# wadewilliamsw1234/Multi-level-Indoor-SLAM

Measured on AMD Instinct MI355X. Metric: keyframes gated/sec (VPR+kNN+LightGlue verify), higher is better.
Workload: dtype bf16

## Files before the change

### include/mlgate.h

```cpp
#ifndef MLGATE_H
#define MLGATE_H

#include <stddef.h>
#include <stdint.h>

#ifdef __cplusplus
extern "C" {
#endif

#define MLG_OK 0
#define MLG_EINVAL (-1)
#define MLG_EHIP (-2)
#define MLG_ENOMEM (-3)

#define MLG_VIT_DEPTH 12
#define MLG_VIT_EMBED 768
#define MLG_VIT_PATCH_K 768

#define MLG_ABI_VERSION 3
#define MLG_STRUCT_INIT(T) {(uint32_t)sizeof(T), (uint32_t)MLG_ABI_VERSION}
int mlg_abi_version(void);
const char* mlg_strerror(int status);

typedef struct mlg_vit_block {
// ... 263 lines not shown

typedef struct mlg_lg_block {
    const uint16_t* Wqkv; const float* bqkv;
    const uint16_t* Wout; const float* bout;
    const uint16_t* Wf1;  const float* bf1;
    const float* ln_g;    const float* ln_b;
    const uint16_t* Wf2;  const float* bf2;
} mlg_lg_block;
typedef struct mlg_lg_weights {
    uint32_t struct_size, abi_version;
    const float* Wr;
    mlg_lg_block self[9], cross[9];
    const uint16_t* Wfinal[9]; const float* bfinal[9];
    const float* wmatch[9];    const float* bmatch[9];
    const float* wconf[8];     const float* bconf[8];
    const float* ones;
} mlg_lg_weights;
size_t mlg_lightglue_workspace_bytes(int P, int kmax);
int mlg_lightglue(const mlg_lg_weights* w, const float* keypoints, const float* descriptors, const int32_t* counts,
                  int F, int kmax, const int32_t* pair_a, const int32_t* pair_b, int P, float depth_confidence,
                  float width_confidence, float filter_threshold, int pruning_min_kpts, void* workspace,
                  size_t workspace_bytes, int32_t* matches, float* scores, int32_t* num_matches, int32_t* stop_layer,
                  void* stream);

int mlg_lg_orient_matches(const int32_t* matches, const float* scores, const int32_t* num_matches,
                          const int32_t* rows, const uint8_t* swap, int P, int kmax, int32_t* matches_out,
                          float* scores_out, int32_t* num_out, void* stream);

int mlg_dbg_lg_trace_begin(void* dev_buf, size_t bytes);
int mlg_dbg_lg_trace_end(int32_t* tags, int32_t* counts, int max_entries);
int mlg_dbg_fill_lds(uint32_t pattern, void* sink, void* stream);
int mlg_dbg_fill_regs(uint32_t pattern, void* stream);
int mlg_dbg_ransac_poison_nsol(int on, int value);
int mlg_dbg_ffn_trace(void* host, size_t bytes);
int mlg_dbg_att_trace(void* host, size_t bytes);

typedef struct mlg_sg_weights {
    uint32_t struct_size, abi_version;
    const float* kenc_w[3]; const float* kenc_b[3];
    const uint16_t* kenc_w4; const float* kenc_b4;
    const uint16_t* kenc_w5; const float* kenc_b5;
    mlg_lg_block layer[18];
    const uint16_t* Wfinal; const float* bfinal;
    float bin_score;
} mlg_sg_weights;
size_t mlg_superglue_workspace_bytes(int P, int kmax);
int mlg_superglue(const mlg_sg_weights* w, const float* keypoints, const float* scores, const float* descriptors,
                  const int32_t* counts, int F, int kmax, int W, int H, const int32_t* pair_a, const int32_t* pair_b,
                  int P, int sinkhorn_iterations, float match_threshold, void* workspace, size_t workspace_bytes,
                  int32_t* matches, float* match_scores, int32_t* num_matches, void* stream);

size_t mlg_ransac_workspace_bytes(int P, long S_total, int hypotheses);
int mlg_ransac_epipolar(const float* kp1, const float* kp2, const int32_t* offsets, int P, long S_total,
                        const double* K, int k_stride, double threshold, int hypotheses, uint64_t seed,
                        void* workspace, size_t workspace_bytes, double* model, uint8_t* mask, int32_t* inliers,
                        double* pose, int32_t* status, void* stream);
int mlg_recover_pose(const float* kp1, const float* kp2, const int32_t* offsets, int P, const double* K,
                     int k_stride, const double* E, const uint8_t* mask, double* pose, void* stream);

#define MLG_LOFTR_NCONV 21
typedef struct {
    const uint16_t* w;
    const uint16_t* wmerge;
    const uint16_t* w1;
    const uint16_t* w2;
    const float *ln1_g, *ln1_b, *ln2_g, *ln2_b;
// ... 80 lines not shown
```

### multi-level-indoor-slam_amd/csrc/ransac.hip

```cpp
#include "common.h"
#include "kernels.h"
#include "ws_carve.h"

#define RS_FN __host__ __device__ static inline
#define RS_CONST static __constant__ const
#include "rs_math.h"

namespace {

#define RS_HD __host__ __device__

constexpr int MAXSOL = 10;
constexpr int RS_CHUNK = 1024;
constexpr int RS_ROUND1 = 256;

__device__ __forceinline__ int nsol_at(const int8_t* __restrict__ nsol, size_t i) {
    return min(max((int)nsol[i], 0), MAXSOL);
}


template <int MR>
RS_HD bool null_space9(double (&A)[MR][9], double (&N)[9 - MR][9]) {
    int piv_col[MR];
    int r = 0;
    for (int c = 0; c < 9 && r < MR; ++c) {
        int best = r;
        double bv = fabs(A[r][c]);
        for (int i = r + 1; i < MR; ++i)
            if (fabs(A[i][c]) > bv) { bv = fabs(A[i][c]); best = i; }
        if (bv < 1e-12) continue;
        if (best != r)
            for (int j = 0; j < 9; ++j) { double t = A[r][j]; A[r][j] = A[best][j]; A[best][j] = t; }
        const double inv = 1.0 / A[r][c];
        for (int j = 0; j < 9; ++j) A[r][j] *= inv;
        for (int i = 0; i < MR; ++i)
            if (i != r) {
                const double f = A[i][c];
                if (f != 0.0)
                    for (int j = 0; j < 9; ++j) A[i][j] -= f * A[r][j];
            }
        piv_col[r++] = c;
    }
    if (r < MR) return false;
    bool is_piv[9] = {false, false, false, false, false, false, false, false, false};
    for (int i = 0; i < MR; ++i) is_piv[piv_col[i]] = true;
    int k = 0;
    for (int f = 0; f < 9; ++f) {
// ... 480 lines not shown
        }
        if (__all(done)) break;
    }
    bool real = r < n && fabs(zi) <= 1e-7 * fmax(1.0, fabs(zr));
    double x = zr;
    if (real) {
#pragma unroll
        for (int pass = 0; pass < 2; ++pass) {
            double f = 0.0, df = 0.0;
#pragma unroll
            for (int i = 10; i >= 0; --i)
                if (i <= n) { df = df * x + f; f = f * x + c[i]; }
            if (df != 0.0) {
                const double xn = x - f / df;
                if (isfinite(xn)) x = xn;
            }
        }
    }
    int nn = 0;
#pragma unroll
    for (int j = 0; j < 10; ++j) {
        const double v = __shfl(x, gl + j, 64);
        const int isr = __shfl((int)real, gl + j, 64);
        if (isr) {
#pragma unroll
            for (int i = 0; i < 10; ++i)
                if (i == nn) roots[i] = v;
            ++nn;
        }
    }
    return nn;
}

__device__ __forceinline__ bool hyp5_active(const PairInfo& pi, int h, int H, const int32_t* __restrict__ nsub, int p) {
    return h < H && (pi.mode == 5 ? h == 0 : h < nsub[p]);
}

__device__ __forceinline__ bool hyp5_null(const PairInfo& pi, const double4* __restrict__ ptsn,
                                          const int32_t* __restrict__ subsets, int p, int H, int h,
                                          double (&Nb)[4][9]) {
    double q1[5][2], q2[5][2];
    for (int i = 0; i < 5; ++i) {
        const int id = pi.mode == 5 ? i : subsets[((size_t)p * H + h) * 7 + i];
        const double4 q = ptsn[pi.start + id];
        q1[i][0] = q.x; q1[i][1] = q.y; q2[i][0] = q.z; q2[i][1] = q.w;
    }
    double A[5][9];
    for (int i = 0; i < 5; ++i) {
        const double x1 = q1[i][0], y1 = q1[i][1], x2 = q2[i][0], y2 = q2[i][1];
        A[i][0] = x2 * x1; A[i][1] = x2 * y1; A[i][2] = x2;
        A[i][3] = y2 * x1; A[i][4] = y2 * y1; A[i][5] = y2;
        A[i][6] = x1;      A[i][7] = y1;      A[i][8] = 1.0;
    }
    return null_space5_reg(A, Nb);
}

__global__ __launch_bounds__(64) void k_ransac_null5(const PairInfo* __restrict__ info, const double4* __restrict__ ptsn,
                                                     int H, const int32_t* __restrict__ subsets,
                                                     const int32_t* __restrict__ nsub, double* __restrict__ models,
                                                     int h0, int hn, const uint8_t* __restrict__ done) {
    const int p = blockIdx.y;
    const int h = h0 + blockIdx.x * 64 + threadIdx.x;
    if (h >= h0 + hn || (done && done[p])) return;
    const PairInfo pi = info[p];
    if (!(pi.mode == 1 || pi.mode == 5) || !hyp5_active(pi, h, H, nsub, p)) return;
    double Nb[4][9];
    const bool ok = hyp5_null(pi, ptsn, subsets, p, H, h, Nb);
    double* o = models + ((size_t)p * H + h) * MAXSOL * 9;
#pragma unroll
    for (int a = 0; a < 4; ++a)
#pragma unroll
        for (int k = 0; k < 9; ++k) o[9 * a + k] = Nb[a][k];
    o[36] = ok ? 1.0 : 0.0;
}

constexpr int HYP5_GS = 10, HYP5_GPW = 64 / HYP5_GS, HYP5_GPB = 4 * HYP5_GPW;
constexpr int SLOT_FLAG = 36, SLOT_POLY = 37, SLOT_MAT = 48;
constexpr double FLAG_POLY = 2.0;

template <class BX, class BY, class B1, class NB>
__device__ __forceinline__ int hyp5_models(const double (&zr)[10], int nz, BX bx, BY by, B1 b1, NB nb,
                                           double* __restrict__ out) {
    int ns = 0;
#pragma unroll
    for (int t = 0; t < 10; ++t) {
        if (t >= nz) continue;
        const double z = zr[t];
        double M[3][3];
#pragma unroll
        for (int i = 0; i < 3; ++i) {
            double vx = 0.0, vy = 0.0, v1 = 0.0;
#pragma unroll
            for (int d = 3; d >= 0; --d) { vx = vx * z + bx(i, d); vy = vy * z + by(i, d); }
#pragma unroll
            for (int d = 4; d >= 0; --d) v1 = v1 * z + b1(i, d);
            M[i][0] = vx; M[i][1] = vy; M[i][2] = v1;
        }
        double best[3] = {0.0, 0.0, 0.0}, bn = -1.0;
#pragma unroll
        for (int a = 0; a < 3; ++a) {
            const int b = (a + 1) % 3;
            const double cx = M[a][1] * M[b][2] - M[a][2] * M[b][1];
            const double cy = M[a][2] * M[b][0] - M[a][0] * M[b][2];
            const double cz = M[a][0] * M[b][1] - M[a][1] * M[b][0];
            const double n2 = cx * cx + cy * cy + cz * cz;
            if (n2 > bn) { bn = n2; best[0] = cx; best[1] = cy; best[2] = cz; }
        }
        if (!(fabs(best[2]) > 1e-300 * sqrt(fmax(bn, 1e-300)))) continue;
        const double x = best[0] / best[2], y = best[1] / best[2];
        if (!(fabs(x) < 1e300) || !(fabs(y) < 1e300)) continue;
        double e[9], nrm = 0.0;
#pragma unroll
        for (int k = 0; k < 9; ++k) {
            e[k] = x * nb(0, k) + y * nb(1, k) + z * nb(2, k) + nb(3, k);
            nrm += e[k] * e[k];
        }
        nrm = 1.0 / sqrt(nrm);
        double* Eo = out + ns * 9;
#pragma unroll
        for (int k = 0; k < 9; ++k) Eo[k] = e[k] * nrm;
        ++ns;
    }
    return ns;
}

__global__ __launch_bounds__(256) void k_ransac_hyp5(const PairInfo* __restrict__ info,
                                                     const double4* __restrict__ ptsn, int H,
                                                     const int32_t* __restrict__ subsets,
                                                     const int32_t* __restrict__ nsub, double* __restrict__ models,
                                                     int8_t* __restrict__ nsol, int h0,
                                                     const uint8_t* __restrict__ done) {
    constexpr int GS = HYP5_GS, GPW = HYP5_GPW, GPB = HYP5_GPB;
    __shared__ double snb[GPB][4][9];
    const int lane = threadIdx.x & 63, gw = lane / GS;
    const bool valid = gw < GPW;
    const int g = (threadIdx.x >> 6) * GPW + (valid ? gw : 0), r = lane - gw * GS, gl = gw * GS;
    const int p = blockIdx.y;
    const int h = h0 + blockIdx.x * GPB + g;
    if (done && done[p]) return;
    const PairInfo pi = info[p];
    const bool ess = pi.mode == 1 || pi.mode == 5;
    const bool act = valid && ess && hyp5_active(pi, h, H, nsub, p);
    if (!ess) return;
    bool ok = act;
    if (act) {
        const double* nb = models + ((size_t)p * H + h) * MAXSOL * 9;
        for (int i = r; i < 36; i += GS) snb[g][i / 9][i % 9] = nb[i];
        ok = nb[36] != 0.0;
    }
    __syncthreads();
    if (!valid) return;
#if defined(RS_ABLATE) && RS_ABLATE == 3
    if (act && r == 0) nsol[(size_t)p * H + h] = 0;
    return;
#endif
    auto ent = [&](int k, double* l) {
        for (int a = 0; a < 4; ++a) l[a] = snb[g][a][k];
    };
    double row[20];
#pragma unroll
    for (int j = 0; j < 20; ++j) row[j] = 0.0;
    if (ok && r == 0) {
        const int cof[3][5] = {{0, 4, 8, 5, 7}, {1, 3, 8, 5, 6}, {2, 3, 7, 4, 6}};
        const double sg[3] = {1.0, -1.0, 1.0};
#pragma unroll
        for (int t = 0; t < 3; ++t) {
            double l0[4], l1[4], l2[4], l3[4], l4[4];
            ent(cof[t][0], l0); ent(cof[t][1], l1); ent(cof[t][2], l2); ent(cof[t][3], l3); ent(cof[t][4], l4);
            double q[10];
#pragma unroll
            for (int s = 0; s < 10; ++s) q[s] = 0.0;
            q_fma(q, l1, l2, sg[t]);
            q_fma(q, l3, l4, -sg[t]);
            c_fma(row, q, l0);
        }
// ... 43 lines not shown
            if (ob > best) { best = ob; bl = jl; }
        }
        if (!(best > 1e-300)) ok = false;
        piv[c] = bl;
        double prow[20];
#pragma unroll
        for (int jj = c; jj < 20; ++jj) prow[jj] = __shfl(row[jj], gl + bl, 64);
        const double inv = ok ? 1.0 / prow[c] : 0.0;
        if (r == bl) {
#pragma unroll
            for (int jj = c; jj < 20; ++jj) row[jj] = prow[jj] * inv;
            used = true;
        } else {
            const double f = row[c] * inv;
#pragma unroll
            for (int jj = c; jj < 20; ++jj) row[jj] -= f * prow[jj];
        }
    }
    double bx[3][4], by[3][4], b1[3][5];
#pragma unroll
    for (int i = 0; i < 3; ++i) {
        double a4[10], a5[10];
#pragma unroll
        for (int k = 0; k < 10; ++k) {
            a4[k] = __shfl(row[10 + k], gl + piv[4 + 2 * i], 64);
            a5[k] = __shfl(row[10 + k], gl + piv[5 + 2 * i], 64);
        }
        bx[i][0] = a4[2]; bx[i][1] = a4[1] - a5[2]; bx[i][2] = a4[0] - a5[1]; bx[i][3] = -a5[0];
        by[i][0] = a4[5]; by[i][1] = a4[4] - a5[5]; by[i][2] = a4[3] - a5[4]; by[i][3] = -a5[3];
        b1[i][0] = a4[9]; b1[i][1] = a4[8] - a5[9]; b1[i][2] = a4[7] - a5[8]; b1[i][3] = a4[6] - a5[7];
        b1[i][4] = -a5[6];
    }
    if (!ok) {
        if (h < H && r == 0) nsol[(size_t)p * H + h] = 0;
        return;
    }
#if defined(RS_ABLATE) && RS_ABLATE == 2
    if (r == 0) nsol[(size_t)p * H + h] = (int8_t)(bx[0][0] > 1e300);
    return;
#endif
    double poly[11];
#pragma unroll
    for (int i = 0; i < 11; ++i) poly[i] = 0.0;
    {
        double t[8];
#pragma unroll
        for (int i = 0; i < 8; ++i) t[i] = 0.0;
        pmul_acc<4, 5>(t, by[1], b1[2], 1.0);
        pmul_acc<5, 4>(t, b1[1], by[2], -1.0);
        pmul_acc<4, 8>(poly, bx[0], t, 1.0);
#pragma unroll
        for (int i = 0; i < 8; ++i) t[i] = 0.0;
        pmul_acc<4, 5>(t, bx[1], b1[2], 1.0);
        pmul_acc<5, 4>(t, b1[1], bx[2], -1.0);
        pmul_acc<4, 8>(poly, by[0], t, -1.0);
        double u[7];
#pragma unroll
        for (int i = 0; i < 7; ++i) u[i] = 0.0;
        pmul_acc<4, 4>(u, bx[1], by[2], 1.0);
        pmul_acc<4, 4>(u, by[1], bx[2], -1.0);
        pmul_acc<5, 7>(poly, b1[0], u, 1.0);
    }
#if defined(RS_ABLATE) && RS_ABLATE == 1
    if (r == 0) nsol[(size_t)p * H + h] = (int8_t)(poly[3] > 1e300);
    return;
#endif
    if (r == 0) {
        double* o = models + ((size_t)p * H + h) * MAXSOL * 9;
#pragma unroll
        for (int i = 0; i < 11; ++i) o[SLOT_POLY + i] = poly[i];
#pragma unroll
        for (int i = 0; i < 3; ++i) {
#pragma unroll
            for (int d = 0; d < 4; ++d) {
                o[SLOT_MAT + 13 * i + d] = bx[i][d];
                o[SLOT_MAT + 13 * i + 4 + d] = by[i][d];
            }
#pragma unroll
            for (int d = 0; d < 5; ++d) o[SLOT_MAT + 13 * i + 8 + d] = b1[i][d];
        }
        o[SLOT_FLAG] = FLAG_POLY;
    }
}

__global__ __launch_bounds__(256) void k_ransac_roots5(const PairInfo* __restrict__ info, int H,
                                                       const int32_t* __restrict__ nsub, double* __restrict__ models,
                                                       int8_t* __restrict__ nsol, int h0,
                                                       const uint8_t* __restrict__ done) {
    constexpr int GS = HYP5_GS, GPW = HYP5_GPW, GPB = HYP5_GPB;
    __shared__ double2 szs[GPB][17];
    __shared__ double scoef[GPB][39 + 36];
    const int lane = threadIdx.x & 63, gw = lane / GS;
    const bool valid = gw < GPW;
    const int g = (threadIdx.x >> 6) * GPW + (valid ? gw : 0), r = lane - gw * GS, gl = gw * GS;
    const int p = blockIdx.y;
    const int h = h0 + blockIdx.x * GPB + g;
    if (done && done[p]) return;
    const PairInfo pi = info[p];
    if (!(pi.mode == 1 || pi.mode == 5) || !valid || !hyp5_active(pi, h, H, nsub, p)) return;
    double* o = models + ((size_t)p * H + h) * MAXSOL * 9;
    if (o[SLOT_FLAG] != FLAG_POLY) return;
    double* sc = scoef[g];
    for (int i = r; i < 39; i += GS) sc[i] = o[SLOT_MAT + i];
    for (int i = r; i < 36; i += GS) sc[39 + i] = o[i];
    double poly[11], zr[10];
#pragma unroll
    for (int i = 0; i < 11; ++i) poly[i] = o[SLOT_POLY + i];
    const int nz = real_roots10(poly, zr, r, gl, szs[g]);
    if (r != 0) return;
    __builtin_amdgcn_wave_barrier();
    nsol[(size_t)p * H + h] = (int8_t)hyp5_models(
        zr, nz, [&](int i, int d) { return sc[13 * i + d]; }, [&](int i, int d) { return sc[13 * i + 4 + d]; },
        [&](int i, int d) { return sc[13 * i + 8 + d]; }, [&](int a, int k) { return sc[39 + 9 * a + k]; }, o);
}

__global__ __launch_bounds__(64) void k_ransac_subsets(const PairInfo* __restrict__ info, int P, int H,
                                                       const float* __restrict__ kp1, const float* __restrict__ kp2,
                                                       int32_t* __restrict__ subsets, int32_t* __restrict__ nsub) {
    const int p = blockIdx.x * blockDim.x + threadIdx.x;
    if (p >= P) return;
    const PairInfo pi = info[p];
    if (pi.mode != 1 && pi.mode != 2) {
        nsub[p] = 0;
        return;
    }
    const int m = pi.mode == 1 ? 5 : 7;
    CvRng rng{~0ull};
    int32_t* out = subsets + (size_t)p * H * 7;
    int it = 0;
    for (; it < H; ++it) {
        int idx[7];
        float a[7][2], b[7][2];
        int iters = 0, i = 0;
        for (; iters < RANSAC_MAX_ATTEMPTS; ++iters) {
            for (i = 0; i < m;) {
                int v;
                for (;;) {
                    v = idx[i] = rng.uniform(0, pi.count);
                    int j = 0;
                    for (; j < i; ++j)
                        if (v == idx[j]) break;
                    if (j == i) break;
                }
                a[i][0] = kp1[2 * (pi.start + v)]; a[i][1] = kp1[2 * (pi.start + v) + 1];
                b[i][0] = kp2[2 * (pi.start + v)]; b[i][1] = kp2[2 * (pi.start + v) + 1];
                ++i;
            }
            if (m == 7 && (collinear_last(a, 7) || collinear_last(b, 7))) continue;
            break;
        }
        if (!(i == m && iters < RANSAC_MAX_ATTEMPTS)) break;
        for (int j = 0; j < m; ++j) out[it * 7 + j] = idx[j];
    }
    nsub[p] = it;
}

__global__ __launch_bounds__(64) void k_ransac_hyp(const PairInfo* __restrict__ info, const double4* __restrict__ ptsn,
                                                   int H, uint64_t seed, const int32_t* __restrict__ subsets,
                                                   const int32_t* __restrict__ nsub, double* __restrict__ models,
                                                   int8_t* __restrict__ nsol, int h0, const uint8_t* __restrict__ done) {
    const int p = blockIdx.y;
    const int h = h0 + blockIdx.x * blockDim.x + threadIdx.x;
    if (h >= H || (done && done[p])) return;
    const PairInfo pi = info[p];
    double* out = models + ((size_t)p * H + h) * MAXSOL * 9;
    if (pi.mode == 1 || pi.mode == 5) return;
    const bool direct = pi.mode == 4;
    if (pi.mode == 0 || (direct && h > 0)) {
        nsol[(size_t)p * H + h] = 0;
        return;
    }
    int idx[7];
    if (direct) {
        for (int i = 0; i < 7; ++i) idx[i] = i;
    } else if (pi.mode == 2) {
        if (h >= nsub[p]) {
            nsol[(size_t)p * H + h] = 0;
            return;
        }
        for (int i = 0; i < 7; ++i) idx[i] = subsets[((size_t)p * H + h) * 7 + i];
    } else {
        uint64_t st = splitmix(seed ^ (uint64_t)h * 0x632BE59BD9B4E019ull);
        for (int i = 0; i < 7; ++i) {
            int v;
            bool dup;
            do {
                st = splitmix(st);
                v = (int)((st >> 11) % (uint64_t)pi.count);
                dup = false;
                for (int j = 0; j < i; ++j) dup |= idx[j] == v;
            } while (dup);
            idx[i] = v;
        }
    }
    double q1[7][2], q2[7][2];
    for (int i = 0; i < 7; ++i) {
        const double4 q = ptsn[pi.start + idx[i]];
        q1[i][0] = q.x; q1[i][1] = q.y; q2[i][0] = q.z; q2[i][1] = q.w;
    }
    double Fn[3 * 9];
    const int ns = solve_7pt(q1, q2, Fn);
    for (int s = 0; s < ns; ++s) denorm_F(Fn + s * 9, pi.T1, pi.T2, out + s * 9);
    nsol[(size_t)p * H + h] = (int8_t)ns;
}

__global__ __launch_bounds__(256) void k_ransac_score(const PairInfo* __restrict__ info, const double4* __restrict__ ptsn,
                                                      const double4* __restrict__ ptsr, int H,
                                                      const double* __restrict__ models,
                                                      const int8_t* __restrict__ nsol, float* __restrict__ score,
                                                      int h0, const uint8_t* __restrict__ done) {
    __shared__ double4 sp[RS_CHUNK];
    const int p = blockIdx.y;
    const int h = h0 + blockIdx.x * blockDim.x + threadIdx.x;
    if (done && done[p]) return;
    const PairInfo pi = info[p];
    if (pi.mode == 0) {
        if (h < H)
            for (int s = 0; s < MAXSOL; ++s) score[((size_t)p * H + h) * MAXSOL + s] = -INFINITY;
        return;
    }
    const bool ess = pi.mode == 1 || pi.mode == 5;
    const double4* src = (ess ? ptsn : ptsr) + pi.start;
    const int ns = h < H ? nsol_at(nsol, (size_t)p * H + h) : 0;
    int cnt[MAXSOL];
    for (int s = 0; s < MAXSOL; ++s) cnt[s] = 0;
    const float t2 = (float)pi.thr2;
    const double t2_hi = 0.5 * ((double)t2 + (double)nextafterf(t2, INFINITY));
    const double* mh = models + ((size_t)p * H + (h < H ? h : 0)) * MAXSOL * 9;
    if (pi.mode == 3) {
        for (int s = 0; s < MAXSOL; ++s) {
            float med = INFINITY;
            if (s < ns) {
                float e[16];
                for (int i = 0; i < pi.count; ++i) {
                    const double4 q = src[i];
                    e[i] = err_epiline(mh + s * 9, q.x, q.y, q.z, q.w);
                }
                for (int i = 1; i < pi.count; ++i) {
                    const float v = e[i];
                    int j = i - 1;
                    while (j >= 0 && e[j] > v) { e[j + 1] = e[j]; --j; }
                    e[j + 1] = v;
                }
                med = e[pi.count / 2];
            }
            if (h < H) score[((size_t)p * H + h) * MAXSOL + s] = s < ns ? -med : -INFINITY;
        }
        return;
    }
    for (int c0 = 0; c0 < pi.count; c0 += RS_CHUNK) {
        const int cn = min(RS_CHUNK, pi.count - c0);
        __syncthreads();
        for (int i = threadIdx.x; i < cn; i += blockDim.x) sp[i] = src[c0 + i];
        __syncthreads();
        for (int s = 0; s < ns; ++s) {
            double M[9];
            for (int k = 0; k < 9; ++k) M[k] = mh[s * 9 + k];
            int c = 0;
            if (ess) {
                for (int i = 0; i < cn; ++i) {
                    const double4 q = sp[i];
                    c += sampson_inlier(M, q.x, q.y, q.z, q.w, t2, t2_hi);
                }
            } else {
                for (int i = 0; i < cn; ++i) {
                    const double4 q = sp[i];
                    c += err_epiline(M, q.x, q.y, q.z, q.w) <= t2;
                }
            }
            cnt[s] += c;
        }
    }
    if (h < H)
        for (int s = 0; s < MAXSOL; ++s)
            score[((size_t)p * H + h) * MAXSOL + s] = s < ns ? (float)cnt[s] : -INFINITY;
}

RS_HD void jacobi3(double (&A)[3][3], double (&V)[3][3], double (&w)[3]) {
    for (int i = 0; i < 3; ++i)
        for (int j = 0; j < 3; ++j) V[i][j] = i == j ? 1.0 : 0.0;
    for (int sweep = 0; sweep < 50; ++sweep) {
        const double off = fabs(A[0][1]) + fabs(A[0][2]) + fabs(A[1][2]);
        if (off < 1e-300) break;
        for (int p = 0; p < 2; ++p)
            for (int q = p + 1; q < 3; ++q) {
                if (fabs(A[p][q]) < 1e-300) continue;
                const double th = (A[q][q] - A[p][p]) / (2.0 * A[p][q]);
                const double t = (th >= 0 ? 1.0 : -1.0) / (fabs(th) + sqrt(th * th + 1.0));
                const double c = 1.0 / sqrt(t * t + 1.0), s = t * c;
                for (int k = 0; k < 3; ++k) {
                    const double akp = A[k][p], akq = A[k][q];
                    A[k][p] = c * akp - s * akq;
                    A[k][q] = s * akp + c * akq;
                }
                for (int k = 0; k < 3; ++k) {
                    const double apk = A[p][k], aqk = A[q][k];
                    A[p][k] = c * apk - s * aqk;
                    A[q][k] = s * apk + c * aqk;
                }
                for (int k = 0; k < 3; ++k) {
                    const double vkp = V[k][p], vkq = V[k][q];
                    V[k][p] = c * vkp - s * vkq;
                    V[k][q] = s * vkp + c * vkq;
                }
            }
    }
    for (int i = 0; i < 3; ++i) w[i] = A[i][i];
}
// ... 81 lines not shown
    for (int i = 0; i < 4; ++i)
        for (int j = 0; j <= i; ++j) {
            double s = M[i][j];
            for (int k = 0; k < j; ++k) s -= L[i][k] * L[j][k];
            if (i == j) {
                L[i][i] = sqrt(fmax(s, 1e-300));
            } else {
                L[i][j] = s / L[j][j];
            }
        }
    double X[4] = {0.5, 0.5, 0.5, 0.5};
    for (int it = 0; it < 6; ++it) {
        double y[4];
        for (int i = 0; i < 4; ++i) {
            double s = X[i];
            for (int k = 0; k < i; ++k) s -= L[i][k] * y[k];
            y[i] = s / L[i][i];
        }
        for (int i = 3; i >= 0; --i) {
            double s = y[i];
            for (int k = i + 1; k < 4; ++k) s -= L[k][i] * X[k];
            X[i] = s / L[i][i];
        }
        double n = sqrt(X[0] * X[0] + X[1] * X[1] + X[2] * X[2] + X[3] * X[3]);
        for (int i = 0; i < 4; ++i) X[i] /= n;
    }
    if (!(X[2] * X[3] > 0)) return false;
    const double X0 = X[0] / X[3], X1 = X[1] / X[3], X2 = X[2] / X[3];
    if (!(X2 < dist)) return false;
    const double z2 = R[2][0] * X0 + R[2][1] * X1 + R[2][2] * X2 + t[2];
    return z2 > 0 && z2 < dist;
}

__global__ __launch_bounds__(256) void k_ransac_probe(const PairInfo* __restrict__ info, int P, int H, int H1,
                                                      const float* __restrict__ score,
                                                      const int8_t* __restrict__ nsol,
                                                      const int32_t* __restrict__ nsub, uint8_t* __restrict__ done) {
    const int p = blockIdx.x * blockDim.x + threadIdx.x;
    if (p >= P) return;
    const PairInfo pi = info[p];
    uint8_t d = 0;
    if (pi.mode == 1 || pi.mode == 2) {
        const int mp = pi.mode == 1 ? 5 : 7;
        const int ns_it = nsub[p], total = H * MAXSOL;
        int niters = H, max_good = 0;
        for (int it = 0; it < niters && it < ns_it && it < H1; ++it) {
            const int ns = nsol_at(nsol, (size_t)p * H + it);
            for (int s = 0; s < ns; ++s) {
                const int g = (int)score[(size_t)p * total + it * MAXSOL + s];
                if (g > max(max_good, mp - 1)) {
                    max_good = g;
                    niters = ransac_update_iters(RANSAC_CONFIDENCE, (double)(pi.count - g) / pi.count, mp, niters);
                }
            }
        }
        d = (niters <= H1 || ns_it <= H1) ? 1 : 0;
    }
    done[p] = d;
}

__global__ __launch_bounds__(256) void k_ransac_select(const PairInfo* __restrict__ info,
                                                       const double4* __restrict__ ptsn,
                                                       const double4* __restrict__ ptsr, int H,
                                                       const double* __restrict__ models,
                                                       const float* __restrict__ score, const int8_t* __restrict__ nsol,
                                                       const int32_t* __restrict__ nsub, double* __restrict__ model_out,
                                                       uint8_t* __restrict__ mask, int32_t* __restrict__ inliers,
                                                       int32_t* __restrict__ status) {
    const int p = blockIdx.x, tid = threadIdx.x;
    const PairInfo pi = info[p];
    __shared__ float bs[256];
    __shared__ int bi[256];
    __shared__ double Mb[9];
    __shared__ int cnt_sh;
    const int total = H * MAXSOL;
    if (pi.mode == 1 || pi.mode == 2) {
        if (tid == 0) {
            const int mp = pi.mode == 1 ? 5 : 7;
            const int ns_it = nsub[p];
            int niters = H, max_good = 0, bidx = -1;
            for (int it = 0; it < niters && it < ns_it; ++it) {
                const int ns = nsol_at(nsol, (size_t)p * H + it);
                for (int s = 0; s < ns; ++s) {
                    const int g = (int)score[(size_t)p * total + it * MAXSOL + s];
                    if (g > max(max_good, mp - 1)) {
                        max_good = g;
                        bidx = it * MAXSOL + s;
                        niters = ransac_update_iters(RANSAC_CONFIDENCE, (double)(pi.count - g) / pi.count, mp, niters);
                    }
// ... 101 lines not shown
    double nt[3] = {-tv[0], -tv[1], -tv[2]};
    int g[4] = {0, 0, 0, 0};
    for (int i = tid; i < S; i += 256) {
        if (!mask[s0 + i]) continue;
        const double x1 = (kp1[2 * (s0 + i)] - cx) / fx, y1 = (kp1[2 * (s0 + i) + 1] - cy) / fy;
        const double x2 = (kp2[2 * (s0 + i)] - cx) / fx, y2 = (kp2[2 * (s0 + i) + 1] - cy) / fy;
        g[0] += cheiral(R1, tv, x1, y1, x2, y2, 50.0);
        g[1] += cheiral(R2, tv, x1, y1, x2, y2, 50.0);
        g[2] += cheiral(R1, nt, x1, y1, x2, y2, 50.0);
        g[3] += cheiral(R2, nt, x1, y1, x2, y2, 50.0);
    }
    for (int k = 0; k < 4; ++k) atomicAdd(&good[k], g[k]);
    __syncthreads();
    if (tid == 0) {
        const int a = good[0], b = good[1], cc = good[2], d = good[3];
        int pick;
        if (a >= b && a >= cc && a >= d) pick = 0;
        else if (b >= a && b >= cc && b >= d) pick = 1;
        else if (cc >= a && cc >= b && cc >= d) pick = 2;
        else pick = 3;
        const double (*R)[3] = (pick & 1) ? R2 : R1;
        const double* tt = (pick & 2) ? nt : tv;
        double* T = pose + p * 16;
        for (int i = 0; i < 3; ++i) {
            for (int j = 0; j < 3; ++j) T[i * 4 + j] = R[i][j];
            T[i * 4 + 3] = tt[i];
        }
        T[12] = 0.0; T[13] = 0.0; T[14] = 0.0; T[15] = 1.0;
    }
}

bool g_poison_nsol = false;
int g_poison_value = 0;

__global__ __launch_bounds__(64) void k_ransac_poison_nsol(const PairInfo* __restrict__ info, int H,
                                                           const int32_t* __restrict__ nsub, int8_t* __restrict__ nsol,
                                                           int h0, int hn, const uint8_t* __restrict__ done, int value) {
    const int p = blockIdx.y;
    const int h = h0 + blockIdx.x * blockDim.x + threadIdx.x;
    if (h >= h0 + hn || h >= H || (done && done[p])) return;
    const int mode = info[p].mode;
    const bool unused = mode == 0 || ((mode == 4 || mode == 5) && h > 0) || ((mode == 1 || mode == 2) && h >= nsub[p]);
    if (unused) nsol[(size_t)p * H + h] = (int8_t)value;
}

struct RsBufs {
    PairInfo* info;
    double4 *ptsn, *ptsr;
    double* models;
    int8_t* nsol;
    float* score;
    int32_t *subsets, *nsub;
    uint8_t* done;
};

size_t rs_carve(int P, long S_total, int H, void* base, RsBufs* out) {
    WsCarver c(base);
    RsBufs b;
    const size_t PH = (size_t)P * H;
    b.info = c.take<PairInfo>((size_t)P);
    b.ptsn = c.take<double4>((size_t)S_total);
    b.ptsr = c.take<double4>((size_t)S_total);
    b.models = c.take<double>(9 * MAXSOL * PH);
    b.nsol = c.take<int8_t>(PH);
    b.score = c.take<float>(MAXSOL * PH);
    b.subsets = c.take<int32_t>(7 * PH);
    b.nsub = c.take<int32_t>((size_t)P);
    b.done = c.take<uint8_t>((size_t)P);
    if (out) *out = b;
    return c.total();
}

}

size_t mlg_ransac_ws_bytes(int P, long S_total, int H) {
    if (P <= 0 || S_total < 0 || H <= 0) return 0;
    return rs_carve(P, S_total, H, nullptr, nullptr);
}

int mlg_ransac_run(const float* kp1, const float* kp2, const int32_t* offs, int P, long S_total, const double* K,
                   int k_stride, double thr, int H, uint64_t seed, void* ws, size_t ws_bytes, double* model_out,
                   uint8_t* mask, int32_t* inliers, double* pose, int32_t* status, hipStream_t s) {
    if (P <= 0 || H <= 0 || H > (1 << 20) || !(thr > 0.0) || S_total < 0) return MLG_EINVAL;
    RsBufs b;
    if (rs_carve(P, S_total, H, ws, &b) > ws_bytes) return MLG_EINVAL;
    hipLaunchKernelGGL(k_ransac_prep, dim3(P), dim3(256), 0, s, kp1, kp2, offs, K, k_stride, thr, b.info, b.ptsn,
                       b.ptsr);
    MLG_LAUNCH_CHECK();
    hipLaunchKernelGGL(k_ransac_subsets, dim3((P + 63) / 64), dim3(64), 0, s, b.info, P, H, kp1, kp2, b.subsets,
                       b.nsub);
    MLG_LAUNCH_CHECK();
    const int H1 = std::min(H, RS_ROUND1);
    for (int round = 0; round < 2; ++round) {
        const int h0 = round ? H1 : 0, hn = round ? H - H1 : H1;
        const uint8_t* skip = round ? b.done : nullptr;
        if (hn <= 0) break;
        hipLaunchKernelGGL(k_ransac_hyp, dim3((hn + 63) / 64, P), dim3(64), 0, s, b.info, b.ptsn, H, seed, b.subsets,
                           b.nsub, b.models, b.nsol, h0, skip);
        MLG_LAUNCH_CHECK();
        hipLaunchKernelGGL(k_ransac_null5, dim3((hn + 63) / 64, P), dim3(64), 0, s, b.info, b.ptsn, H, b.subsets,
                           b.nsub, b.models, h0, hn, skip);
        MLG_LAUNCH_CHECK();
        hipLaunchKernelGGL(k_ransac_hyp5, dim3((hn + HYP5_GPB - 1) / HYP5_GPB, P), dim3(256), 0, s, b.info, b.ptsn, H,
                           b.subsets, b.nsub, b.models, b.nsol, h0, skip);
        MLG_LAUNCH_CHECK();
        hipLaunchKernelGGL(k_ransac_roots5, dim3((hn + HYP5_GPB - 1) / HYP5_GPB, P), dim3(256), 0, s, b.info, H, b.nsub,
                           b.models, b.nsol, h0, skip);
        MLG_LAUNCH_CHECK();
        if (g_poison_nsol) {
            hipLaunchKernelGGL(k_ransac_poison_nsol, dim3((hn + 63) / 64, P), dim3(64), 0, s, b.info, H, b.nsub, b.nsol,
                               h0, hn, skip, g_poison_value);
            MLG_LAUNCH_CHECK();
        }
        hipLaunchKernelGGL(k_ransac_score, dim3((hn + 255) / 256, P), dim3(256), 0, s, b.info, b.ptsn, b.ptsr, H,
                           b.models, b.nsol, b.score, h0, skip);
        MLG_LAUNCH_CHECK();
        if (round == 0 && H1 < H) {
            hipLaunchKernelGGL(k_ransac_probe, dim3((P + 255) / 256), dim3(256), 0, s, b.info, P, H, H1, b.score,
                               b.nsol, b.nsub, b.done);
            MLG_LAUNCH_CHECK();
        }
    }
    hipLaunchKernelGGL(k_ransac_select, dim3(P), dim3(256), 0, s, b.info, b.ptsn, b.ptsr, H, b.models, b.score, b.nsol,
                       b.nsub, model_out, mask, inliers, status);
    MLG_LAUNCH_CHECK();
    if (pose && K) {
        hipLaunchKernelGGL(k_recover_pose, dim3(P), dim3(256), 0, s, kp1, kp2, offs, K, k_stride, model_out, mask, pose,
                           status);
        MLG_LAUNCH_CHECK();
    }
    return MLG_OK;
}

int mlg_recover_pose_run(const float* kp1, const float* kp2, const int32_t* offs, int P, const double* K,
                         int k_stride, const double* E, const uint8_t* mask, double* pose, hipStream_t s) {
    if (P <= 0) return MLG_EINVAL;
    hipLaunchKernelGGL(k_recover_pose, dim3(P), dim3(256), 0, s, kp1, kp2, offs, K, k_stride, E, mask, pose,
                       (int32_t*)nullptr);
    MLG_LAUNCH_CHECK();
    return MLG_OK;
}

extern "C" int mlg_dbg_ransac_poison_nsol(int on, int value) {
    g_poison_nsol = on != 0;
    g_poison_value = value;
    return MLG_OK;
}
```

### multi-level-indoor-slam_amd/mlgate/_native.py

```python
import ctypes
import os

_HERE = os.path.dirname(os.path.abspath(__file__))
LIB_PATH = os.path.join(_HERE, "libmlgate.so")
TORCH_LIB_PATH = os.path.join(_HERE, "libmlgate_torch.so")
OPS = ("vit_forward_into", "dino_forward_into", "dino_weights_check", "salad_forward", "knn_gate", "knn_query", "row_normalize", "similarity", "xcorr_score", "xcorr_batch",
       "superpoint",
       "lightglue", "ransac_epipolar", "recover_pose", "resnet50", "loftr_features", "loftr_pack_tails", "loftr_coarse_layer", "loftr_match", "superglue", "pillow_resize_224", "plane_ransac", "proximity",
       "jpeg_pixels", "mixvpr_forward", "mixvpr_head", "mixvpr_preprocess", "vlad", "anyloc_forward", "kmeans_step",
       "crica_forward", "vit_trunk", "crica_pool", "crica_encoder",
       "weights_check", "prof_enable", "prof_reset", "prof_read")


c_int, c_long, c_size_t, c_float, c_double, c_void_p = (
    ctypes.c_int, ctypes.c_long, ctypes.c_size_t, ctypes.c_float, ctypes.c_double, ctypes.c_void_p)

EXPORTS = {
    "mlg_abi_version": (c_int, []),
    "mlg_strerror": (ctypes.c_char_p, [c_int]),
    "mlg_vit_workspace_bytes": (c_size_t, [c_int, c_int]),
    "mlg_vit_forward": (c_int, [c_void_p, c_void_p, c_int, c_int, c_int, c_int, c_long, c_int, c_int, c_void_p,
                                c_size_t, c_void_p, c_void_p, c_void_p]),
    "mlg_dino_workspace_bytes": (c_size_t, [c_int, c_int, c_int]),
    "mlg_dino_forward": (c_int, [c_void_p, c_void_p, c_int, c_int, c_int, c_int, c_long, c_int, c_int, c_void_p,
# ... 80 lines not shown
    "mlg_op_gemm_conv": (c_int, [c_void_p, c_int, c_void_p, c_void_p, c_void_p, c_int, c_void_p, c_int, c_void_p,
                                 c_int, c_int, c_int, c_int, c_int, c_int, c_float, c_void_p]),
    "mlg_op_gemm_conv_upadd": (c_int, [c_void_p, c_int, c_void_p, c_void_p, c_void_p, c_int, c_int, c_void_p, c_int,
                                       c_int, c_int, c_void_p]),
    "mlg_op_gemm_bias_relu": (c_int, [c_void_p, c_int, c_void_p, c_void_p, c_void_p, c_int, c_int, c_int, c_int,
                                      c_int, c_void_p]),
    "mlg_op_gemm_bias_add_relu": (c_int, [c_void_p, c_int, c_void_p, c_void_p, c_void_p, c_void_p, c_int, c_void_p,
                                          c_int, c_int, c_int, c_void_p]),
    "mlg_op_gemm_bias_f32_ld": (c_int, [c_void_p, c_int, c_void_p, c_void_p, c_void_p, c_int, c_int, c_int, c_int,
                                        c_void_p]),
    "mlg_op_gemm_bias_split": (c_int, [c_void_p, c_int, c_void_p, c_void_p, c_void_p, c_void_p, c_int, c_int, c_int,
                                       c_void_p]),
    "mlg_op_gemm_qkv": (c_int, [c_void_p] * 6 + [c_int, c_int, c_int, c_void_p]),
    "mlg_op_gemm_patch": (c_int, [c_void_p] * 5 + [c_int, c_int, c_int, c_void_p]),
    "mlg_op_gemm_sim_split_loftr": (c_int, [c_void_p, c_void_p, c_int, c_int, c_int, c_void_p, c_int, c_int, c_int,
                                            c_long, c_void_p]),
    "mlg_op_lg_ffn_ex": (c_int, [c_void_p, c_void_p, c_void_p, c_int, c_int] + [c_void_p] * 8 + [c_int]
                         + [c_void_p] * 5 + [c_float, c_float, c_void_p, c_void_p, c_void_p]),
    "mlg_op_preprocess_patches": (c_int, [c_void_p, c_int, c_int, c_int, c_int, c_long, c_int, c_void_p,
                                          c_void_p]),
    "mlg_prof_enable": (c_int, [c_int]),
    "mlg_prof_reset": (c_int, []),
    "mlg_prof_read": (c_int, [c_int, ctypes.POINTER(c_double), ctypes.POINTER(c_long)]),
    "mlg_prof_read_work": (c_int, [c_int, ctypes.POINTER(c_double)]),
    "mlg_lg_orient_matches": (c_int, [c_void_p] * 5 + [c_int, c_int] + [c_void_p] * 4),
    "mlg_xcorr_batch_workspace_bytes": (c_size_t, [c_int, c_int, c_int, c_int]),
    "mlg_xcorr_batch": (c_int, [c_void_p, c_int, c_int, c_int, c_void_p, c_void_p, c_int, c_void_p, c_size_t,
                                c_void_p, c_void_p]),
    "mlg_dbg_lg_trace_begin": (c_int, [c_void_p, c_size_t]),
    "mlg_dbg_lg_trace_end": (c_int, [c_void_p, c_void_p, c_int]),
    "mlg_dbg_fill_lds": (c_int, [ctypes.c_uint32, c_void_p, c_void_p]),
    "mlg_dbg_fill_regs": (c_int, [ctypes.c_uint32, c_void_p]),
    "mlg_dbg_ransac_poison_nsol": (c_int, [c_int, c_int]),
    "mlg_loftr_tails_bytes": (c_size_t, []),
    "mlg_loftr_pack_tails": (c_int, [c_void_p, c_void_p, c_void_p]),
    "mlg_op_loftr_coarse_layer_ws_bytes": (c_size_t, [c_int, c_int]),
    "mlg_op_loftr_coarse_layer": (c_int, [c_void_p, c_int, c_int, c_void_p, c_void_p, c_int, c_int, c_void_p, c_size_t,
                                          c_void_p]),
    "mlg_png_info": (c_int, [c_void_p, c_size_t, c_void_p, c_void_p, c_void_p, c_void_p]),
    "mlg_png_decode_bgr": (c_int, [c_void_p, c_void_p, c_int, c_void_p, c_int, c_int, c_int, c_void_p]),
    "mlg_png_load_bgr": (c_int, [c_void_p, c_int, c_void_p, c_int, c_int, c_int, c_void_p]),
    "mlg_jpeg_info": (c_int, [c_void_p, c_size_t, c_void_p]),
    "mlg_jpeg_coef_bytes": (c_size_t, [c_int, c_int]),
    "mlg_jpeg_coefs_decode": (c_int, [c_void_p, c_void_p, c_int, c_void_p, c_void_p, c_void_p, c_int, c_int, c_int,
                                      c_void_p]),
    "mlg_jpeg_coefs_load": (c_int, [c_void_p, c_int, c_void_p, c_void_p, c_void_p, c_int, c_int, c_int, c_void_p]),
    "mlg_jpeg_params_check": (c_int, [c_void_p, c_int, c_int, c_int, c_size_t]),
    "mlg_jpeg_pixels": (c_int, [c_void_p, c_void_p, c_void_p, c_int, c_int, c_int, c_void_p, c_void_p]),
}

_lib = None
_ops = None


class MlgateError(RuntimeError):
    pass


def lib():
    global _lib
    if _lib is None:
        if not os.path.exists(LIB_PATH):
            raise MlgateError(f"{LIB_PATH} is missing: build it with `python -c 'import __graft_entry__ as g; "
                              "g.build()'` (hipcc --offload-arch=gfx950)")
        L = ctypes.CDLL(LIB_PATH)
        for name, (res, args) in EXPORTS.items():
# ... 59 lines not shown
```

Before: 545.1.

## Add tiny first RANSAC round and compact scoring over active solutions

RANSAC hypothesis generation and scoring now run in up to three rounds (16, 256, H) rather than two, so pairs that reach their adaptive termination early skip more of the hypothesis work. The scoring kernel builds a per-block prefix-sum list of (hypothesis, solution) items so each thread scores one model over all points, instead of each thread looping over its variable solution count. The aim is less wasted work and less warp divergence. The cost is an extra set of kernel launches plus a probe for the added round, and extra shared-memory bookkeeping in scoring.

```diff
diff --git a/include/mlgate.h b/include/mlgate.h
--- a/include/mlgate.h
+++ b/include/mlgate.h
@@ -319,6 +319,7 @@
 int mlg_dbg_fill_lds(uint32_t pattern, void* sink, void* stream);
 int mlg_dbg_fill_regs(uint32_t pattern, void* stream);
 int mlg_dbg_ransac_poison_nsol(int on, int value);
+int mlg_dbg_ransac_round0(int r0);
 int mlg_dbg_ffn_trace(void* host, size_t bytes);
 int mlg_dbg_att_trace(void* host, size_t bytes);
 
diff --git a/multi-level-indoor-slam_amd/csrc/ransac.hip b/multi-level-indoor-slam_amd/csrc/ransac.hip
--- a/multi-level-indoor-slam_amd/csrc/ransac.hip
+++ b/multi-level-indoor-slam_amd/csrc/ransac.hip
@@ -1,5 +1,6 @@
 #include "common.h"
 #include "kernels.h"
+#include "ransac_rounds.h"
 #include "ws_carve.h"
 
 #define RS_FN __host__ __device__ static inline
@@ -12,7 +13,6 @@
 
 constexpr int MAXSOL = 10;
 constexpr int RS_CHUNK = 1024;
-constexpr int RS_ROUND1 = 256;
 
 __device__ __forceinline__ int nsol_at(const int8_t* __restrict__ nsol, size_t i) {
     return min(max((int)nsol[i], 0), MAXSOL);
@@ -559,8 +559,9 @@
     return nn;
 }
 
-__device__ __forceinline__ bool hyp5_active(const PairInfo& pi, int h, int H, const int32_t* __restrict__ nsub, int p) {
-    return h < H && (pi.mode == 5 ? h == 0 : h < nsub[p]);
+__device__ __forceinline__ bool hyp5_active(const PairInfo& pi, int h, int hend, const int32_t* __restrict__ nsub,
+                                            int p) {
+    return h < hend && (pi.mode == 5 ? h == 0 : h < nsub[p]);
 }
 
 __device__ __forceinline__ bool hyp5_null(const PairInfo& pi, const double4* __restrict__ ptsn,
@@ -590,7 +591,7 @@
     const int h = h0 + blockIdx.x * 64 + threadIdx.x;
     if (h >= h0 + hn || (done && done[p])) return;
     const PairInfo pi = info[p];
-    if (!(pi.mode == 1 || pi.mode == 5) || !hyp5_active(pi, h, H, nsub, p)) return;
+    if (!(pi.mode == 1 || pi.mode == 5) || !hyp5_active(pi, h, h0 + hn, nsub, p)) return;
     double Nb[4][9];
     const bool ok = hyp5_null(pi, ptsn, subsets, p, H, h, Nb);
     double* o = models + ((size_t)p * H + h) * MAXSOL * 9;
@@ -655,7 +656,7 @@
                                                      const double4* __restrict__ ptsn, int H,
                                                      const int32_t* __restrict__ subsets,
                                                      const int32_t* __restrict__ nsub, double* __restrict__ models,
-                                                     int8_t* __restrict__ nsol, int h0,
+                                                     int8_t* __restrict__ nsol, int h0, int hend,
                                                      const uint8_t* __restrict__ done) {
     constexpr int GS = HYP5_GS, GPW = HYP5_GPW, GPB = HYP5_GPB;
     __shared__ double snb[GPB][4][9];
@@ -667,7 +668,7 @@
     if (done && done[p]) return;
     const PairInfo pi = info[p];
     const bool ess = pi.mode == 1 || pi.mode == 5;
-    const bool act = valid && ess && hyp5_active(pi, h, H, nsub, p);
+    const bool act = valid && ess && hyp5_active(pi, h, hend, nsub, p);
     if (!ess) return;
     bool ok = act;
     if (act) {
@@ -777,7 +778,7 @@
         b1[i][4] = -a5[6];
     }
     if (!ok) {
-        if (h < H && r == 0) nsol[(size_t)p * H + h] = 0;
+        if (h < hend && r == 0) nsol[(size_t)p * H + h] = 0;
         return;
     }
 #if defined(RS_ABLATE) && RS_ABLATE == 2
@@ -830,7 +831,7 @@
 
 __global__ __launch_bounds__(256) void k_ransac_roots5(const PairInfo* __restrict__ info, int H,
                                                        const int32_t* __restrict__ nsub, double* __restrict__ models,
-                                                       int8_t* __restrict__ nsol, int h0,
+                                                       int8_t* __restrict__ nsol, int h0, int hend,
                                                        const uint8_t* __restrict__ done) {
     constexpr int GS = HYP5_GS, GPW = HYP5_GPW, GPB = HYP5_GPB;
     __shared__ double2 szs[GPB][17];
@@ -842,7 +843,7 @@
     const int h = h0 + blockIdx.x * GPB + g;
     if (done && done[p]) return;
     const PairInfo pi = info[p];
-    if (!(pi.mode == 1 || pi.mode == 5) || !valid || !hyp5_active(pi, h, H, nsub, p)) return;
+    if (!(pi.mode == 1 || pi.mode == 5) || !valid || !hyp5_active(pi, h, hend, nsub, p)) return;
     double* o = models + ((size_t)p * H + h) * MAXSOL * 9;
     if (o[SLOT_FLAG] != FLAG_POLY) return;
     double* sc = scoef[g];
@@ -903,10 +904,11 @@
 __global__ __launch_bounds__(64) void k_ransac_hyp(const PairInfo* __restrict__ info, const double4* __restrict__ ptsn,
                                                    int H, uint64_t seed, const int32_t* __restrict__ subsets,
                                                    const int32_t* __restrict__ nsub, double* __restrict__ models,
-                                                   int8_t* __restrict__ nsol, int h0, const uint8_t* __restrict__ done) {
+                                                   int8_t* __restrict__ nsol, int h0, int hend,
+                                                   const uint8_t* __restrict__ done) {
     const int p = blockIdx.y;
     const int h = h0 + blockIdx.x * blockDim.x + threadIdx.x;
-    if (h >= H || (done && done[p])) return;
+    if (h >= hend || (done && done[p])) return;
     const PairInfo pi = info[p];
     double* out = models + ((size_t)p * H + h) * MAXSOL * 9;
     if (pi.mode == 1 || pi.mode == 5) return;
@@ -953,26 +955,27 @@
                                                       const double4* __restrict__ ptsr, int H,
                                                       const double* __restrict__ models,
                                                       const int8_t* __restrict__ nsol, float* __restrict__ score,
-                                                      int h0, const uint8_t* __restrict__ done) {
+                                                      int h0, int hend, const uint8_t* __restrict__ done) {
     __shared__ double4 sp[RS_CHUNK];
-    const int p = blockIdx.y;
-    const int h = h0 + blockIdx.x * blockDim.x + threadIdx.x;
+    __shared__ uint16_t items[256 * MAXSOL];
+    __shared__ int wave_items[4];
+    const int p = blockIdx.y, tid = threadIdx.x;
+    const int hb = h0 + blockIdx.x * 256, h = hb + tid;
+    const bool mine = h < hend;
     if (done && done[p]) return;
     const PairInfo pi = info[p];
+    float* sh = score + ((size_t)p * H + (mine ? h : 0)) * MAXSOL;
     if (pi.mode == 0) {
-        if (h < H)
-            for (int s = 0; s < MAXSOL; ++s) score[((size_t)p * H + h) * MAXSOL + s] = -INFINITY;
+        if (mine)
+            for (int s = 0; s < MAXSOL; ++s) sh[s] = -INFINITY;
         return;
     }
     const bool ess = pi.mode == 1 || pi.mode == 5;
     const double4* src = (ess ? ptsn : ptsr) + pi.start;
-    const int ns = h < H ? nsol_at(nsol, (size_t)p * H + h) : 0;
-    int cnt[MAXSOL];
-    for (int s = 0; s < MAXSOL; ++s) cnt[s] = 0;
-    const float t2 = (float)pi.thr2;
-    const double t2_hi = 0.5 * ((double)t2 + (double)nextafterf(t2, INFINITY));
-    const double* mh = models + ((size_t)p * H + (h < H ? h : 0)) * MAXSOL * 9;
+    const int ns = mine ? nsol_at(nsol, (size_t)p * H + h) : 0;
     if (pi.mode == 3) {
+        if (!mine) return;
+        const double* mh = models + ((size_t)p * H + h) * MAXSOL * 9;
         for (int s = 0; s < MAXSOL; ++s) {
             float med = INFINITY;
             if (s < ns) {
@@ -989,19 +992,47 @@
                 }
                 med = e[pi.count / 2];
             }
-            if (h < H) score[((size_t)p * H + h) * MAXSOL + s] = s < ns ? -med : -INFINITY;
+            sh[s] = s < ns ? -med : -INFINITY;
         }
         return;
     }
-    for (int c0 = 0; c0 < pi.count; c0 += RS_CHUNK) {
-        const int cn = min(RS_CHUNK, pi.count - c0);
-        __syncthreads();
-        for (int i = threadIdx.x; i < cn; i += blockDim.x) sp[i] = src[c0 + i];
-        __syncthreads();
-        for (int s = 0; s < ns; ++s) {
-            double M[9];
-            for (int k = 0; k < 9; ++k) M[k] = mh[s * 9 + k];
-            int c = 0;
+    const int lane = tid & 63, wave = tid >> 6;
+    int incl = ns;
+    for (int o = 1; o < 64; o <<= 1) {
+        const int v = __shfl_up(incl, o, 64);
+        if (lane >= o) incl += v;
+    }
+    if (lane == 63) wave_items[wave] = incl;
+    __syncthreads();
+    int first = incl - ns, n_items = 0;
+    for (int w = 0; w < 4; ++w) {
+        if (w < wave) first += wave_items[w];
+        n_items += wave_items[w];
+    }
+    for (int s = 0; s < ns; ++s) items[first + s] = (uint16_t)(tid << 4 | s);
+    if (mine)
+        for (int s = ns; s < MAXSOL; ++s) sh[s] = -INFINITY;
+    __syncthreads();
+    const float t2 = (float)pi.thr2;
+    const double t2_hi = 0.5 * ((double)t2 + (double)nextafterf(t2, INFINITY));
+    const int nchunks = (pi.count + RS_CHUNK - 1) / RS_CHUNK;
+    for (int i0 = 0; i0 < n_items; i0 += 256) {
+        const bool have = i0 + tid < n_items;
+        const int item = have ? items[i0 + tid] : 0;
+        const size_t slot = ((size_t)p * H + hb + (item >> 4)) * MAXSOL + (item & 15);
+        double M[9];
+        if (have)
+            for (int k = 0; k < 9; ++k) M[k] = models[slot * 9 + k];
+        int c = 0;
+        for (int ch = 0; ch < nchunks; ++ch) {
+            if (nchunks > 1 || i0 == 0) {
+                const int c0 = ch * RS_CHUNK;
+                __syncthreads();
+                for (int i = tid; i < min(RS_CHUNK, pi.count - c0); i += 256) sp[i] = src[c0 + i];
+                __syncthreads();
+            }
+            if (!have) continue;
+            const int cn = min(RS_CHUNK, pi.count - ch * RS_CHUNK);
             if (ess) {
                 for (int i = 0; i < cn; ++i) {
                     const double4 q = sp[i];
@@ -1013,12 +1044,9 @@
                     c += err_epiline(M, q.x, q.y, q.z, q.w) <= t2;
                 }
             }
-            cnt[s] += c;
-        }
-    }
-    if (h < H)
-        for (int s = 0; s < MAXSOL; ++s)
-            score[((size_t)p * H + h) * MAXSOL + s] = s < ns ? (float)cnt[s] : -INFINITY;
+        }
+        if (have) score[slot] = (float)c;
+    }
 }
 
 RS_HD void jacobi3(double (&A)[3][3], double (&V)[3][3], double (&w)[3]) {
@@ -1166,19 +1194,19 @@
     return z2 > 0 && z2 < dist;
 }
 
-__global__ __launch_bounds__(256) void k_ransac_probe(const PairInfo* __restrict__ info, int P, int H, int H1,
-                                                      const float* __restrict__ score,
+__global__ __launch_bounds__(256) void k_ransac_probe(const PairInfo* __restrict__ info, int P, int H, int Hr,
+                                                      bool first, const float* __restrict__ score,
                                                       const int8_t* __restrict__ nsol,
                                                       const int32_t* __restrict__ nsub, uint8_t* __restrict__ done) {
     const int p = blockIdx.x * blockDim.x + threadIdx.x;
-    if (p >= P) return;
+    if (p >= P || (!first && done[p])) return;
     const PairInfo pi = info[p];
     uint8_t d = 0;
     if (pi.mode == 1 || pi.mode == 2) {
         const int mp = pi.mode == 1 ? 5 : 7;
         const int ns_it = nsub[p], total = H * MAXSOL;
         int niters = H, max_good = 0;
-        for (int it = 0; it < niters && it < ns_it && it < H1; ++it) {
+        for (int it = 0; it < niters && it < ns_it && it < Hr; ++it) {
             const int ns = nsol_at(nsol, (size_t)p * H + it);
             for (int s = 0; s < ns; ++s) {
                 const int g = (int)score[(size_t)p * total + it * MAXSOL + s];
@@ -1188,7 +1216,7 @@
                 }
             }
         }
-        d = (niters <= H1 || ns_it <= H1) ? 1 : 0;
+        d = (niters <= Hr || ns_it <= Hr) ? 1 : 0;
     }
     done[p] = d;
 }
@@ -1356,6 +1384,7 @@
 
 bool g_poison_nsol = false;
 int g_poison_value = 0;
+int g_round0 = RS_ROUND0;
 
 __global__ __launch_bounds__(64) void k_ransac_poison_nsol(const PairInfo* __restrict__ info, int H,
                                                            const int32_t* __restrict__ nsub, int8_t* __restrict__ nsol,
@@ -1414,22 +1443,22 @@
     hipLaunchKernelGGL(k_ransac_subsets, dim3((P + 63) / 64), dim3(64), 0, s, b.info, P, H, kp1, kp2, b.subsets,
                        b.nsub);
     MLG_LAUNCH_CHECK();
-    const int H1 = std::min(H, RS_ROUND1);
-    for (int round = 0; round < 2; ++round) {
-        const int h0 = round ? H1 : 0, hn = round ? H - H1 : H1;
+    int edges[RS_MAX_ROUNDS];
+    const int rounds = rs_round_edges(H, g_round0, edges);
+    for (int round = 0; round < rounds; ++round) {
+        const int h0 = round ? edges[round - 1] : 0, hend = edges[round], hn = hend - h0;
         const uint8_t* skip = round ? b.done : nullptr;
-        if (hn <= 0) break;
         hipLaunchKernelGGL(k_ransac_hyp, dim3((hn + 63) / 64, P), dim3(64), 0, s, b.info, b.ptsn, H, seed, b.subsets,
-                           b.nsub, b.models, b.nsol, h0, skip);
+                           b.nsub, b.models, b.nsol, h0, hend, skip);
         MLG_LAUNCH_CHECK();
         hipLaunchKernelGGL(k_ransac_null5, dim3((hn + 63) / 64, P), dim3(64), 0, s, b.info, b.ptsn, H, b.subsets,
                            b.nsub, b.models, h0, hn, skip);
         MLG_LAUNCH_CHECK();
         hipLaunchKernelGGL(k_ransac_hyp5, dim3((hn + HYP5_GPB - 1) / HYP5_GPB, P), dim3(256), 0, s, b.info, b.ptsn, H,
-                           b.subsets, b.nsub, b.models, b.nsol, h0, skip);
+                           b.subsets, b.nsub, b.models, b.nsol, h0, hend, skip);
         MLG_LAUNCH_CHECK();
         hipLaunchKernelGGL(k_ransac_roots5, dim3((hn + HYP5_GPB - 1) / HYP5_GPB, P), dim3(256), 0, s, b.info, H, b.nsub,
-                           b.models, b.nsol, h0, skip);
+                           b.models, b.nsol, h0, hend, skip);
         MLG_LAUNCH_CHECK();
         if (g_poison_nsol) {
             hipLaunchKernelGGL(k_ransac_poison_nsol, dim3((hn + 63) / 64, P), dim3(64), 0, s, b.info, H, b.nsub, b.nsol,
@@ -1437,11 +1466,11 @@
             MLG_LAUNCH_CHECK();
         }
         hipLaunchKernelGGL(k_ransac_score, dim3((hn + 255) / 256, P), dim3(256), 0, s, b.info, b.ptsn, b.ptsr, H,
-                           b.models, b.nsol, b.score, h0, skip);
+                           b.models, b.nsol, b.score, h0, hend, skip);
         MLG_LAUNCH_CHECK();
-        if (round == 0 && H1 < H) {
-            hipLaunchKernelGGL(k_ransac_probe, dim3((P + 255) / 256), dim3(256), 0, s, b.info, P, H, H1, b.score,
-                               b.nsol, b.nsub, b.done);
+        if (round + 1 < rounds) {
+            hipLaunchKernelGGL(k_ransac_probe, dim3((P + 255) / 256), dim3(256), 0, s, b.info, P, H, hend, round == 0,
+                               b.score, b.nsol, b.nsub, b.done);
             MLG_LAUNCH_CHECK();
         }
     }
@@ -1470,3 +1499,8 @@
     g_poison_value = value;
     return MLG_OK;
 }
+
+extern "C" int mlg_dbg_ransac_round0(int r0) {
+    if (r0 > 0) g_round0 = r0;
+    return g_round0;
+}
diff --git a/multi-level-indoor-slam_amd/csrc/ransac_rounds.h b/multi-level-indoor-slam_amd/csrc/ransac_rounds.h
--- /dev/null
+++ b/multi-level-indoor-slam_amd/csrc/ransac_rounds.h
@@ -0,0 +1,15 @@
+#pragma once
+
+constexpr int RS_ROUND0 = 16;
+constexpr int RS_ROUND1 = 256;
+constexpr int RS_MAX_ROUNDS = 3;
+
+inline int rs_round_edges(int H, int r0, int (&edges)[RS_MAX_ROUNDS]) {
+    const int want[RS_MAX_ROUNDS] = {r0, RS_ROUND1, H};
+    int n = 0, prev = 0;
+    for (int i = 0; i < RS_MAX_ROUNDS; ++i) {
+        const int e = want[i] < H ? want[i] : H;
+        if (e > prev) edges[n++] = prev = e;
+    }
+    return n;
+}
diff --git a/multi-level-indoor-slam_amd/mlgate/_native.py b/multi-level-indoor-slam_amd/mlgate/_native.py
--- a/multi-level-indoor-slam_amd/mlgate/_native.py
+++ b/multi-level-indoor-slam_amd/mlgate/_native.py
@@ -136,6 +136,7 @@
     "mlg_dbg_fill_lds": (c_int, [ctypes.c_uint32, c_void_p, c_void_p]),
     "mlg_dbg_fill_regs": (c_int, [ctypes.c_uint32, c_void_p]),
     "mlg_dbg_ransac_poison_nsol": (c_int, [c_int, c_int]),
+    "mlg_dbg_ransac_round0": (c_int, [c_int]),
     "mlg_loftr_tails_bytes": (c_size_t, []),
     "mlg_loftr_pack_tails": (c_int, [c_void_p, c_void_p, c_void_p]),
     "mlg_op_loftr_coarse_layer_ws_bytes": (c_size_t, [c_int, c_int]),
```

After: 548.6 (median of 6 runs). About the same (+0.6%).
